# atoptima/DynamicSparseArrays.jl

Measured on NVIDIA B200. Metric: batched PCSR insert/delete Mupdates/s, higher is better.
Workload: dtype int64 keys / f64 values

## Files before the change

dynamicsparsearrays.jl_b200/csrc/tile.cuh:

```cuda
#pragma once
#include "pcsr.cuh"

namespace dsa {

__global__ void __launch_bounds__(256, 6) k_tile_assign(const int64_t* __restrict__ partkeys, const int64_t* __restrict__ inkeys,
                                                        const double* __restrict__ vals, int64_t n_host, const int64_t* __restrict__ n_dev,
                                                        const int64_t* __restrict__ live_keys, const int32_t* __restrict__ live_slot,
                                                        int64_t nlive, const int32_t* __restrict__ keymap, int64_t keymap_min,
                                                        int64_t keymap_len, const int64_t* __restrict__ keys, int64_t cap,
                                                        const int64_t* __restrict__ sem, const int32_t* __restrict__ next_slot,
                                                        int64_t nslots, int64_t* __restrict__ cs, int32_t* __restrict__ tcnt,
                                                        TileRec* __restrict__ rec) {
    int64_t n = n_host;
    if (n_dev) n = *n_dev < n_host ? *n_dev : n_host;
    if (blockIdx.x == 0 && threadIdx.x == 0) cs[CS_N] = n;
    int64_t mink = INT64_MAX, maxk = INT64_MIN, maxp = INT64_MIN, maxknz = INT64_MIN, minp = INT64_MAX;
    int miss = 0;
    int bmax = 0;
    for (int64_t i = (int64_t)blockIdx.x * blockDim.x + threadIdx.x; i < n; i += (int64_t)gridDim.x * blockDim.x) {
        const int64_t pk = partkeys[i];
        const int64_t k = inkeys[i];
        const double v = vals[i];
        minp = pk < minp ? pk : minp;
        int32_t s;
        if (keymap) {
            const int64_t r = pk - keymap_min;
            s = (r >= 0 && r < keymap_len) ? keymap[r] : -1;
        } else {
            s = live_lookup(live_keys, live_slot, nlive, pk);
        }
        mink = k < mink ? k : mink;
        maxk = k > maxk ? k : maxk;
        const bool is_set = v != 0.0;
        if (is_set) {
            maxp = pk > maxp ? pk : maxp;
            maxknz = k > maxknz ? k : maxknz;
        }
        int64_t ps = -1;
        if (s >= 0) ps = sem[s];
        if (ps < 0) {
            miss += 1;
            continue;
        }
        if (k < 1) continue;
        const int32_t ns = next_slot ? next_slot[s] : (s + 1 < nslots ? s + 1 : -1);
        const int64_t pe = ns >= 0 ? sem[ns] : cap;
        const int64_t from = is_set ? ps + 1 : ps;
        const int64_t to = pe - 1;
        int64_t t = ps >> TILE_LG, lo = from, hi = to;
        const int64_t t_last = to >> TILE_LG;
        if (t != t_last) {
            int64_t blo = t + 1, bhi = t_last;
            while (blo <= bhi) {
                const int64_t u = (blo + bhi) >> 1;
                int64_t p = u << TILE_LG;
                int64_t kk = keys[p];
                while (kk == GAP_KEY && p < to) kk = keys[++p];
                if (kk != GAP_KEY && kk <= k) {
                    t = u;
                    blo = u + 1;
                } else {
                    bhi = u - 1;
                }
            }
            const int64_t tb0 = t << TILE_LG;
            lo = from > tb0 ? from : tb0;
            hi = to < tb0 + TILE_CELLS - 1 ? to : tb0 + TILE_CELLS - 1;
        }
        const int64_t tb = t << TILE_LG;
        const int li = atomicAdd(&tcnt[t * TILE_CNT_STRIDE], 1);
        bmax = li + 1 > bmax ? li + 1 : bmax;
        if (li < TILE_CAP) {
            int4* out = reinterpret_cast<int4*>(rec + t * TILE_CAP + li);
            const uint64_t ku = (uint64_t)k, vu = (uint64_t)__double_as_longlong(v);
            out[0] = make_int4((int)(uint32_t)ku, (int)(uint32_t)(ku >> 32), (int)(uint32_t)vu, (int)(uint32_t)(vu >> 32));
            out[1] = make_int4((int)(uint32_t)i, s, (int)((uint32_t)(lo - tb) | ((uint32_t)(hi - tb) << 16)), 0);
        }
    }
#pragma unroll
    for (int o = 16; o > 0; o >>= 1) {
        int64_t a = __shfl_xor_sync(0xffffffffu, mink, o); mink = a < mink ? a : mink;
        a = __shfl_xor_sync(0xffffffffu, maxk, o); maxk = a > maxk ? a : maxk;
        a = __shfl_xor_sync(0xffffffffu, maxp, o); maxp = a > maxp ? a : maxp;
        a = __shfl_xor_sync(0xffffffffu, maxknz, o); maxknz = a > maxknz ? a : maxknz;
        a = __shfl_xor_sync(0xffffffffu, minp, o); minp = a < minp ? a : minp;
        miss += __shfl_xor_sync(0xffffffffu, miss, o);
        const int b2 = __shfl_xor_sync(0xffffffffu, bmax, o);
        bmax = b2 > bmax ? b2 : bmax;
    }
    __shared__ int64_t sh[5][8];
    __shared__ int shm[8], shb[8];
    const int wid = threadIdx.x >> 5, lane = threadIdx.x & 31;
    if (lane == 0) {
        sh[0][wid] = mink; sh[1][wid] = maxk; sh[2][wid] = maxp; sh[3][wid] = maxknz; sh[4][wid] = minp;
        shm[wid] = miss;
        shb[wid] = bmax;
    }
    __syncthreads();
    if (threadIdx.x == 0) {
        for (int w = 1; w < 8; ++w) {
            mink = sh[0][w] < mink ? sh[0][w] : mink;
            maxk = sh[1][w] > maxk ? sh[1][w] : maxk;
            maxp = sh[2][w] > maxp ? sh[2][w] : maxp;
            maxknz = sh[3][w] > maxknz ? sh[3][w] : maxknz;
            minp = sh[4][w] < minp ? sh[4][w] : minp;
            miss += shm[w];
            bmax = shb[w] > bmax ? shb[w] : bmax;
        }
        unsigned long long* u = (unsigned long long*)cs;
        if (bmax) atomicMax((long long*)&cs[CS_MAXBUCKET], (long long)bmax);
        if (miss) atomicAdd(&u[CS_MISSING], (unsigned long long)miss);
        if (mink != INT64_MAX) atomicMax(&u[CS_MINKEY], ~cs_code(mink));
        if (maxk != INT64_MIN) atomicMax(&u[CS_MAXKEY], cs_code(maxk));
        if (maxp != INT64_MIN) atomicMax(&u[CS_MAXPART_NZ], cs_code(maxp));
        if (maxknz != INT64_MIN) atomicMax(&u[CS_MAXKEY_NZ], cs_code(maxknz));
        if (minp != INT64_MAX) atomicMax(&u[CS_MINPART], ~cs_code(minp));
    }
}

__device__ __forceinline__ unsigned mask_le_c(int x) { return x >= 31 ? 0xffffffffu : ((2u << x) - 1u); }

template <int LGS>
__device__ __forceinline__ int tile_find(const int64_t* sk, const uint32_t* live, const uint16_t* fpos, int64_t key, int lo, int hi,
                                         bool* hit) {
    constexpr int S = 1 << LGS;
    *hit = false;
    if (lo <= hi) {
        int a = lo >> LGS, b = hi >> LGS;
        int best = a;
        ++a;
        while (a <= b) {
            const int mid = (a + b) >> 1;
            const int p = fpos[mid];
            if (p <= hi && sk[p] <= key) {
                best = mid;
                a = mid + 1;
            } else {
                b = mid - 1;
            }
        }
        const int c0 = best << LGS;
        unsigned m = live[best];
        if (lo > c0) m &= ~((1u << (lo - c0)) - 1u);
        if (hi < c0 + S - 1) m &= mask_le_c(hi - c0);
        while (m) {
            const int q = 31 - __clz(m);
            const int64_t k = sk[c0 + q];
            if (k <= key) {
                *hit = k == key;
                return c0 + q;
            }
            m ^= 1u << q;
        }
        hi = lo - 1;
    }
    int i = hi;
    while (i > 0 && sk[i] == GAP_KEY) --i;
    return i < 0 ? 0 : i;
}

__device__ __forceinline__ unsigned mask_le(int x) { return x >= 31 ? 0xffffffffu : ((2u << x) - 1u); }

static_assert(TILE_CAP <= 256 && TILE_CELLS <= 2048, "op indices are stored in 8 bits, tile-local positions in 15");
struct TileSmem {
    int64_t sk[TILE_CELLS];
    int64_t rkey[TILE_CAP];
    double rval[TILE_CAP];
    union {
        struct {
            uint32_t rarr[TILE_CAP];
            int32_t rslot[TILE_CAP];
        } op;
        struct {
            uint16_t code[TILE_CELLS + TILE_MAX_LEAVES];
            uint8_t leaf[TILE_MAX_LEAVES];
        } work;
    } u;
    uint32_t live[TILE_MAX_LEAVES];
    uint32_t del[TILE_MAX_LEAVES];
    uint32_t insm[TILE_MAX_LEAVES];
    int nins[TILE_MAX_LEAVES];
    int lhead[TILE_MAX_LEAVES];
    uint16_t fpos[TILE_MAX_LEAVES];
    uint16_t rpos[TILE_CAP];
    int16_t rnext[TILE_CAP];
    uint8_t rstat[TILE_CAP];
    uint8_t rop[TILE_CELLS];
    int nwork;
};

struct TileArgs {
    int64_t* keys;
    double* vals;
    const TileRec* rec;
    const int32_t* tcnt;
    int64_t* sem;
    const uint8_t* destpos;
    int32_t* leafcnt;
    uint8_t* touched;
    int32_t* inscnt;
    int32_t* ins_first;
    int64_t* ins_key;
    double* ins_val;
    int64_t* ins_pos;
    int64_t* status;
};

__device__ __forceinline__ int tile_insert_rank(const TileSmem& s, int head, int pp, int64_t key) {
    int rk = 0;
    for (int o = head; o >= 0; o = s.rnext[o]) {
        if (s.rstat[o]) {
            const int po = s.rpos[o] & 0x7fff;
            rk += (po < pp) || (po == pp && s.rkey[o] < key);
        }
    }
    return rk;
}

template <int LGS>
__global__ void __launch_bounds__(TILE_THREADS, TILE_CTAS_PER_SM) k_tile_merge(TileArgs A, Levels L) {
    extern __shared__ __align__(16) unsigned char tile_smem_raw[];
    TileSmem& s = *reinterpret_cast<TileSmem*>(tile_smem_raw);
    const int t = blockIdx.x;
    const int tid = threadIdx.x, lane = tid & 31, warp = tid >> 5;
    const int64_t tbase = (int64_t)t << TILE_LG;
    constexpr int lgS = LGS, S = 1 << lgS, NL = TILE_CELLS >> lgS;
    const int mn0 = (int)L.mn[0], mx0 = (int)L.mx[0];
    constexpr unsigned FULL = 0xffffffffu;
    constexpr int ROWS = TILE_CELLS / 32, WARPS = TILE_THREADS / 32, RPW = ROWS / WARPS, OPT = TILE_CAP / TILE_THREADS;
    constexpr int VPT = TILE_CELLS / 2 / TILE_THREADS;

    int nrec = A.tcnt[(int64_t)t * TILE_CNT_STRIDE];
    int4 ra[OPT], rb[OPT];
    {
        const int tp = t + TILE_PREFETCH_DIST;
        if (tp < (int)gridDim.x) {
            const char* pk = reinterpret_cast<const char*>(A.keys + ((int64_t)tp << TILE_LG));
            const char* pr = reinterpret_cast<const char*>(A.rec + (int64_t)tp * TILE_CAP);
            if (tid < TILE_CELLS * 8 / 128) asm volatile("prefetch.global.L2 [%0];" ::"l"(pk + tid * 128));
            else if (tid < TILE_CELLS * 8 / 128 + 24) asm volatile("prefetch.global.L2 [%0];" ::"l"(pr + (tid - TILE_CELLS * 8 / 128) * 128));
        }
        const uint64_t l2pol = l2_evict_first_policy();
        longlong2 kk[VPT];
        const longlong2* gk = reinterpret_cast<const longlong2*>(A.keys + tbase);
#pragma unroll
        for (int i = 0; i < VPT; ++i) kk[i] = ldg_stream2(gk + tid + i * TILE_THREADS, l2pol);
        if (nrec > TILE_CAP) nrec = TILE_CAP;
#pragma unroll
        for (int i = 0; i < OPT; ++i) {
            const int j = tid + i * TILE_THREADS;
            if (j < nrec) {
                const int4* rp = reinterpret_cast<const int4*>(A.rec + (int64_t)t * TILE_CAP + j);
                ra[i] = rp[0];
                rb[i] = rp[1];
            }
        }
        if (nrec <= 0) return;
#pragma unroll
        for (int i = 0; i < VPT; ++i) reinterpret_cast<longlong2*>(s.sk)[tid + i * TILE_THREADS] = kk[i];
        for (int l = tid; l < NL; l += TILE_THREADS) {
            s.del[l] = 0;
            s.insm[l] = 0;
            s.nins[l] = 0;
            s.lhead[l] = -1;
        }
        if (tid == 0) s.nwork = 0;
    }
    __syncthreads();
    {
        constexpr int G = 32 >> lgS;
        constexpr unsigned gmask = S >= 32 ? 0xffffffffu : ((1u << (S & 31)) - 1u);
#pragma unroll
        for (int i = 0; i < RPW; ++i) {
            const int row = i * WARPS + warp;
            const unsigned b = __ballot_sync(FULL, s.sk[(row << 5) + lane] != GAP_KEY);
            if (lane < G) s.live[row * G + lane] = (b >> (lane << lgS)) & gmask;
        }
    }
    __syncthreads();
    for (int l = tid; l < NL; l += TILE_THREADS) {
        const unsigned m = s.live[l];
        int p = (l << lgS) + __ffs(m) - 1;
        if (m == 0) {
            p = (l + 1) << lgS;
            while (p < TILE_CELLS && s.sk[p] == GAP_KEY) ++p;
        }
        s.fpos[l] = (uint16_t)p;
    }
    __syncthreads();

#pragma unroll
    for (int i = 0; i < OPT; ++i) {
        const int j = tid + i * TILE_THREADS;
        if (j < nrec) {
            const int4 a = ra[i], b = rb[i];
            const int64_t key = (int64_t)((uint64_t)(uint32_t)a.x | ((uint64_t)(uint32_t)a.y << 32));
            const int lo = (int)((uint32_t)b.z & 0xffffu), hi = (int)((uint32_t)b.z >> 16);
            bool hit = false;
            const int pos = tile_find<LGS>(s.sk, s.live, s.fpos, key, lo, hi, &hit);
            s.rkey[j] = key;
            s.rval[j] = __longlong_as_double((long long)((uint64_t)(uint32_t)a.z | ((uint64_t)(uint32_t)a.w << 32)));
            s.u.op.rarr[j] = (uint32_t)b.x;
            s.u.op.rslot[j] = b.y;
            s.rpos[j] = (uint16_t)(pos | (hit ? 0x8000 : 0));
            s.rnext[j] = (int16_t)atomicExch(&s.lhead[pos >> lgS], j);
        }
    }
    __syncthreads();

    for (int j = tid; j < nrec; j += TILE_THREADS) {
        const int64_t key = s.rkey[j];
        const int32_t slot = s.u.op.rslot[j];
        const uint32_t arr = s.u.op.rarr[j];
        const int pp = s.rpos[j];
        const int pos = pp & 0x7fff, l = pos >> lgS;
        bool dead = false;
        for (int o = s.lhead[l]; o >= 0; o = s.rnext[o]) dead |= (s.rkey[o] == key && s.u.op.rslot[o] == slot && s.u.op.rarr[o] > arr);
        const double v = s.rval[j];
        uint8_t st = 0;
        if (!dead) {
            if (pp & 0x8000) {
                if (v != 0.0) A.vals[tbase + pos] = v;
                else atomicOr(&s.del[l], 1u << (pos & (S - 1)));
            } else if (v != 0.0) {
                st = 1;
                atomicAdd(&s.nins[l], 1);
                asm volatile("prefetch.global.L2 [%0];" ::"l"(A.vals + tbase + (l << lgS)));
            }
        }
        s.rstat[j] = st;
    }
    __syncthreads();

    for (int j = tid; j < nrec; j += TILE_THREADS) {
        if (!s.rstat[j]) continue;
        const int pp = s.rpos[j] & 0x7fff, l = pp >> lgS;
        const unsigned surv = s.live[l] & ~s.del[l];
        const int m = __popc(surv) + s.nins[l];
        if (m < mn0 || m > mx0) continue;
        const int R = __popc(surv & mask_le(pp & (S - 1))) + tile_insert_rank(s, s.lhead[l], pp, s.rkey[j]);
        s.rop[(l << lgS) + R] = (uint8_t)j;
        atomicOr(&s.insm[l], 1u << R);
    }
    __syncthreads();

    constexpr uint32_t CODE_GAP = 0xffffu, CODE_OP = 0x8000u;
    for (int l = tid; l < NL; l += TILE_THREADS) {
        const int ni = s.nins[l];
        const unsigned dl = s.del[l];
        if (ni == 0 && dl == 0) continue;
        unsigned surv = s.live[l] & ~dl;
        const int cnt = __popc(surv);
        const int m = cnt + ni;
        const bool relay = ni > 0 && m >= mn0 && m <= mx0;
        const int64_t lg = (int64_t)t * NL + l;
        const int lcell = l << lgS;
        A.touched[lg] = 1;
        if (relay) {
            A.leafcnt[lg] = m;
            const int slot = atomicAdd(&s.nwork, 1);
            uint16_t* w = s.u.work.code + slot * (S + 1);
            s.u.work.leaf[slot] = (uint8_t)l;
            const unsigned mask = L.leafmask[m], insm = s.insm[l];
            int r = 0;
#pragma unroll
            for (int q = 0; q < S; ++q) {
                uint32_t code = CODE_GAP;
                if ((mask >> q) & 1u) {
                    if ((insm >> r) & 1u) {
                        code = CODE_OP | s.rop[lcell + r];
                    } else {
                        code = (uint32_t)(__ffs(surv) - 1);
                        surv &= surv - 1;
                    }
                    ++r;
                }
                w[q] = (uint16_t)code;
            }
            continue;
        }
        if (dl) {
            A.leafcnt[lg] = cnt;
            for (unsigned d = dl; d; d &= d - 1) A.keys[tbase + lcell + (__ffs(d) - 1)] = GAP_KEY;
        }
        if (ni) {
            const int head = s.lhead[l];
            const int64_t gb = (int64_t)atomicAdd((unsigned long long*)&A.status[ST_NINS], (unsigned long long)ni);
            for (int j = head; j >= 0; j = s.rnext[j]) {
                if (!s.rstat[j]) continue;
                const int pp = s.rpos[j] & 0x7fff;
                const int rk = tile_insert_rank(s, head, pp, s.rkey[j]);
                A.ins_key[gb + rk] = s.rkey[j];
                A.ins_val[gb + rk] = s.rval[j];
                A.ins_pos[gb + rk] = tbase + pp;
            }
            A.inscnt[lg] = ni;
            A.ins_first[lg] = (int32_t)gb;
        }
    }
    __syncthreads();

    const int nwork = s.nwork << lgS;
    constexpr int EU = 4;
    for (int w0 = 0; w0 < nwork; w0 += EU * TILE_THREADS) {
        int64_t k[EU];
        double v[EU];
        int cell[EU];
#pragma unroll
        for (int u = 0; u < EU; ++u) {
            const int w = w0 + u * TILE_THREADS + tid;
            cell[u] = -1;
            k[u] = GAP_KEY;
            v[u] = 0.0;
            if (w < nwork) {
                const int slot = w >> lgS, q = w & (S - 1);
                const uint32_t code = s.u.work.code[slot * (S + 1) + q];
                const int lcell = (int)s.u.work.leaf[slot] << lgS;
                cell[u] = lcell + q;
                if (code < 32u) {
                    k[u] = s.sk[lcell + (int)code];
                    v[u] = A.vals[tbase + lcell + (int)code];
                } else if (code != CODE_GAP) {
                    k[u] = s.rkey[code & 0xffu];
                    v[u] = s.rval[code & 0xffu];
                }
            }
        }
        __syncwarp();
#pragma unroll
        for (int u = 0; u < EU; ++u) {
            if (cell[u] >= 0) {
                const int64_t p = tbase + cell[u];
                A.keys[p] = k[u];
                A.vals[p] = v[u];
                if (k[u] == 0) A.sem[(int64_t)v[u] - 1] = p;
            }
        }
    }
}

}
```

Baseline: 2244.

## Replace per-leaf relayout code table with warp-cooperative lane-per-cell relayout

Drops the per-leaf serial loop that built a 16-bit code table for each relaid leaf. Relay leaves are now compacted with a warp ballot and each warp processes whole leaves with one lane per cell, deriving the source from popcounts and a small survivor-index table. Surviving values are moved between lanes with shuffles instead of reloaded from global memory. One __syncthreads is removed by merging the insert-rank pass after the leaf pass, at the cost of more complex warp-level indexing. A SASS phase-counting profiling script is also added.

```diff
diff --git a/dynamicsparsearrays.jl_b200/csrc/tile.cuh b/dynamicsparsearrays.jl_b200/csrc/tile.cuh
--- a/dynamicsparsearrays.jl_b200/csrc/tile.cuh
+++ b/dynamicsparsearrays.jl_b200/csrc/tile.cuh
@@ -172,9 +172,10 @@
             int32_t rslot[TILE_CAP];
         } op;
         struct {
-            uint16_t code[TILE_CELLS + TILE_MAX_LEAVES];
-            uint8_t leaf[TILE_MAX_LEAVES];
-        } work;
+            uint2 leaf[TILE_MAX_LEAVES];
+            uint8_t lid[TILE_MAX_LEAVES];
+            uint8_t sidx[TILE_CELLS];
+        } lay;
     } u;
     uint32_t live[TILE_MAX_LEAVES];
     uint32_t del[TILE_MAX_LEAVES];
@@ -186,7 +187,7 @@
     int16_t rnext[TILE_CAP];
     uint8_t rstat[TILE_CAP];
     uint8_t rop[TILE_CELLS];
-    int nwork;
+    int nrelay;
 };
 
 struct TileArgs {
@@ -264,7 +265,7 @@
             s.nins[l] = 0;
             s.lhead[l] = -1;
         }
-        if (tid == 0) s.nwork = 0;
+        if (tid == 0) s.nrelay = 0;
     }
     __syncthreads();
     {
@@ -332,53 +333,26 @@
     }
     __syncthreads();
 
-    for (int j = tid; j < nrec; j += TILE_THREADS) {
-        if (!s.rstat[j]) continue;
-        const int pp = s.rpos[j] & 0x7fff, l = pp >> lgS;
-        const unsigned surv = s.live[l] & ~s.del[l];
-        const int m = __popc(surv) + s.nins[l];
-        if (m < mn0 || m > mx0) continue;
-        const int R = __popc(surv & mask_le(pp & (S - 1))) + tile_insert_rank(s, s.lhead[l], pp, s.rkey[j]);
-        s.rop[(l << lgS) + R] = (uint8_t)j;
-        atomicOr(&s.insm[l], 1u << R);
-    }
-    __syncthreads();
-
-    constexpr uint32_t CODE_GAP = 0xffffu, CODE_OP = 0x8000u;
     for (int l = tid; l < NL; l += TILE_THREADS) {
         const int ni = s.nins[l];
-        const unsigned dl = s.del[l];
+        const unsigned dl = s.del[l], surv = s.live[l] & ~dl;
+        const int cnt = __popc(surv), m = cnt + ni;
+        const bool relay = ni > 0 && m >= mn0 && m <= mx0;
+        const unsigned b = __ballot_sync(FULL, relay);
+        int base = 0;
+        if (lane == 0 && b) base = atomicAdd(&s.nrelay, __popc(b));
+        base = __shfl_sync(FULL, base, 0);
         if (ni == 0 && dl == 0) continue;
-        unsigned surv = s.live[l] & ~dl;
-        const int cnt = __popc(surv);
-        const int m = cnt + ni;
-        const bool relay = ni > 0 && m >= mn0 && m <= mx0;
         const int64_t lg = (int64_t)t * NL + l;
-        const int lcell = l << lgS;
         A.touched[lg] = 1;
         if (relay) {
             A.leafcnt[lg] = m;
-            const int slot = atomicAdd(&s.nwork, 1);
-            uint16_t* w = s.u.work.code + slot * (S + 1);
-            s.u.work.leaf[slot] = (uint8_t)l;
-            const unsigned mask = L.leafmask[m], insm = s.insm[l];
-            int r = 0;
-#pragma unroll
-            for (int q = 0; q < S; ++q) {
-                uint32_t code = CODE_GAP;
-                if ((mask >> q) & 1u) {
-                    if ((insm >> r) & 1u) {
-                        code = CODE_OP | s.rop[lcell + r];
-                    } else {
-                        code = (uint32_t)(__ffs(surv) - 1);
-                        surv &= surv - 1;
-                    }
-                    ++r;
-                }
-                w[q] = (uint16_t)code;
-            }
+            const int i = base + __popc(b & ((1u << lane) - 1u));
+            s.u.lay.leaf[i] = make_uint2(surv, L.leafmask[m]);
+            s.u.lay.lid[i] = (uint8_t)l;
             continue;
         }
+        const int lcell = l << lgS;
         if (dl) {
             A.leafcnt[lg] = cnt;
             for (unsigned d = dl; d; d &= d - 1) A.keys[tbase + lcell + (__ffs(d) - 1)] = GAP_KEY;
@@ -398,42 +372,60 @@
             A.ins_first[lg] = (int32_t)gb;
         }
     }
-    __syncthreads();
-
-    const int nwork = s.nwork << lgS;
-    constexpr int EU = 4;
-    for (int w0 = 0; w0 < nwork; w0 += EU * TILE_THREADS) {
-        int64_t k[EU];
-        double v[EU];
-        int cell[EU];
-#pragma unroll
-        for (int u = 0; u < EU; ++u) {
-            const int w = w0 + u * TILE_THREADS + tid;
-            cell[u] = -1;
-            k[u] = GAP_KEY;
-            v[u] = 0.0;
-            if (w < nwork) {
-                const int slot = w >> lgS, q = w & (S - 1);
-                const uint32_t code = s.u.work.code[slot * (S + 1) + q];
-                const int lcell = (int)s.u.work.leaf[slot] << lgS;
-                cell[u] = lcell + q;
-                if (code < 32u) {
-                    k[u] = s.sk[lcell + (int)code];
-                    v[u] = A.vals[tbase + lcell + (int)code];
-                } else if (code != CODE_GAP) {
-                    k[u] = s.rkey[code & 0xffu];
-                    v[u] = s.rval[code & 0xffu];
+    for (int j = tid; j < nrec; j += TILE_THREADS) {
+        if (!s.rstat[j]) continue;
+        const int pp = s.rpos[j] & 0x7fff, l = pp >> lgS;
+        const unsigned surv = s.live[l] & ~s.del[l];
+        const int m = __popc(surv) + s.nins[l];
+        if (m < mn0 || m > mx0) continue;
+        const int R = __popc(surv & mask_le(pp & (S - 1))) + tile_insert_rank(s, s.lhead[l], pp, s.rkey[j]);
+        s.rop[(l << lgS) + R] = (uint8_t)j;
+        atomicOr(&s.insm[l], 1u << R);
+    }
+    __syncthreads();
+
+    {
+        constexpr int G = 32 >> lgS;
+        const int nrelay = s.nrelay;
+        const int q = lane & (S - 1), g0 = lane & ~(S - 1);
+        const unsigned below = (1u << q) - 1u;
+        int64_t* const kq = A.keys + tbase + q;
+        double* const vq = A.vals + tbase + q;
+        for (int i0 = warp * G; i0 < nrelay; i0 += WARPS * G) {
+            const int i = i0 + (lane >> lgS);
+            const bool on = i < nrelay;
+            uint2 e = make_uint2(0u, 0u);
+            int lcell = 0;
+            double vold = 0.0;
+            if (on) {
+                e = s.u.lay.leaf[i];
+                lcell = (int)s.u.lay.lid[i] << lgS;
+                vold = vq[lcell];
+                if ((e.x >> q) & 1u) s.u.lay.sidx[lcell + __popc(e.x & below)] = (uint8_t)q;
+            }
+            __syncwarp();
+            int64_t k = GAP_KEY;
+            double v = 0.0;
+            int src = -1;
+            if ((e.y >> q) & 1u) {
+                const int r = __popc(e.y & below);
+                const unsigned insm = s.insm[lcell >> lgS];
+                if ((insm >> r) & 1u) {
+                    const int o = s.rop[lcell + r];
+                    k = s.rkey[o];
+                    v = s.rval[o];
+                } else {
+                    const int c = s.u.lay.sidx[lcell + r - __popc(insm & ((1u << r) - 1u))];
+                    k = s.sk[lcell + c];
+                    src = g0 + c;
                 }
             }
-        }
-        __syncwarp();
-#pragma unroll
-        for (int u = 0; u < EU; ++u) {
-            if (cell[u] >= 0) {
-                const int64_t p = tbase + cell[u];
-                A.keys[p] = k[u];
-                A.vals[p] = v[u];
-                if (k[u] == 0) A.sem[(int64_t)v[u] - 1] = p;
+            const double vs = __shfl_sync(FULL, vold, src & 31);
+            if (on) {
+                if (src >= 0) v = vs;
+                kq[lcell] = k;
+                vq[lcell] = v;
+                if (k == 0) A.sem[(int64_t)v - 1] = tbase + lcell + q;
             }
         }
     }
diff --git a/profiles/sass_phases.py b/profiles/sass_phases.py
--- /dev/null
+++ b/profiles/sass_phases.py
@@ -0,0 +1,52 @@
+#!/usr/bin/env python
+import os
+import re
+import subprocess
+import sys
+import tempfile
+from collections import Counter
+
+root = os.path.dirname(os.path.dirname(os.path.abspath(__file__)))
+so = os.path.abspath(sys.argv[1] if len(sys.argv) > 1 else os.path.join(root, "dynamicsparsearrays.jl_b200", "libdsa.so"))
+lines = open(os.path.join(os.path.dirname(so), "csrc", "tile.cuh")).read().splitlines()
+marks = [(i + 1, l.strip()[8:30]) for i, l in enumerate(lines) if l.strip().startswith("// ---- ")]
+kstart = next(i + 1 for i, l in enumerate(lines) if "k_tile_merge(TileArgs" in l)
+cuda = os.environ.get("CUDA_HOME", "/usr/local/cuda")
+
+
+def phase(f, n):
+    if f != "tile.cuh":
+        return f
+    if n < kstart:
+        return "helpers (tile_find, ranks)"
+    p = "prologue"
+    for ln, name in marks:
+        if n >= ln:
+            p = name
+    return p
+
+
+with tempfile.TemporaryDirectory() as tmp:
+    subprocess.check_call([f"{cuda}/bin/cuobjdump", "-xelf", "all", so], cwd=tmp, stdout=subprocess.DEVNULL)
+    cubin = next(os.path.join(tmp, f) for f in os.listdir(tmp) if f.endswith(".cubin"))
+    sass = subprocess.check_output([f"{cuda}/bin/nvdisasm", "-g", "-c", cubin], text=True)
+
+counts, fn, loc = {}, None, None
+for ln in sass.splitlines():
+    m = re.match(r"\s*\.text\.(\S*k_tile_merge\S*):", ln)
+    if m:
+        fn = m.group(1)
+        counts[fn] = Counter()
+        continue
+    if ln.startswith("//---------------------") and "k_tile_merge" not in ln:
+        fn = None
+    m = re.search(r'//## File "([^"]+)", line (\d+)', ln)
+    if m:
+        loc = (os.path.basename(m.group(1)), int(m.group(2)))
+    elif fn and loc and re.match(r"\s+/\*[0-9a-f]{4,}\*/", ln):
+        counts[fn][phase(*loc)] += 1
+for fn in sorted(counts):
+    c = counts[fn]
+    print(f"{fn}: {sum(c.values())} static SASS instructions")
+    for k, v in sorted(c.items(), key=lambda kv: -kv[1]):
+        print(f"  {v:5d}  {k}")
```

Measured after the change: 2364 (median of 6 runs). 5.3% higher.
